# AwesomePeiweiPan/Droid-SLAM_Reserch

Hardware: AMD Instinct MI355X
Metric: BA update iters/sec (2000-edge equivalents; 256 keyframes, 48x64) (higher is better)
Workload: dtype f32; 1 GPU; 256-keyframe / 2000-edge global BA, 48x64, t0=1, lm=1e-5 ep=1e-2 (BASELINE configs[2]); edges_total=2000, solve=fp64 dense Cholesky on device, chol_failed=False

## Files before the change

droid-slam_reserch_amd/csrc/api.hip:

```cpp
#include <hip/hip_runtime.h>
#include <stdarg.h>
#include <stdio.h>

#include <map>
#include <mutex>

#include "../../include/droid_backends_hip.h"
#include "ba_internal.hpp"
#include "graph.hpp"

namespace droid {
int launch_corr_index_forward(const void* volume, const float* coords, void* corr, int B, int H1,
                              int W1, int H2, int W2, int r, int dtype, hipStream_t s);
int launch_corr_pyramid_forward(const void* const* volumes, const float* coords, void* corr, int B, int H1, int W1,
                                int r, int levels, int dtype, hipStream_t s);
int launch_corr_pyramid_forward_slots(const void* const* volumes, const int64_t* slots, long long cap, const float* coords,
                                      void* corr, int B, int H1, int W1, int r, int levels, int dtype, hipStream_t s);
int launch_corr_index_backward(const float* coords, const void* corr_grad, void* volume_grad, int B,
                               int H1, int W1, int H2, int W2, int r, int dtype, hipStream_t s);
int launch_altcorr_pyramid_forward(const void* const* levels_dev, const int64_t* ii, const int64_t* jj,
                                   const float* coords, float* corr, int E, int frames, int H, int W, int C,
                                   int r, int nlevels, int dtype, hipStream_t s);
int launch_altcorr_forward(const void* f1, const void* f2, const float* coords, void* corr, int B,
                           int N, int H1, int W1, int H2, int W2, int C, int r, int dtype,
// ... 483 lines not shown
int droid_ba_status(const void* workspace, void* stream, int* status_out, int* depth_slots_out) {
  if (!workspace) return fail(DROID_E_ARG, "ba_status: null %s", "workspace");
  int hdr[HDR_WORDS];
  hipError_t e = hipMemcpyAsync(hdr, workspace, sizeof(hdr), hipMemcpyDeviceToHost, (hipStream_t)stream);
  if (e == hipSuccess) e = hipStreamSynchronize((hipStream_t)stream);
  if (e != hipSuccess) {
    snprintf(g_err, sizeof(g_err), "ba_status: %s", hipGetErrorString(e));
    return DROID_E_HIP;
  }
  if (status_out) *status_out = hdr[HDR_STATUS];
  if (depth_slots_out) *depth_slots_out = hdr[HDR_M];
  return DROID_OK;
}

int droid_ba_attach_launch_hints(const void* workspace, int* hints) {
  if (!workspace) return fail(DROID_E_ARG, "ba_attach_launch_hints: null %s", "workspace");
  std::lock_guard<std::mutex> lock(g_mirror_mu);
  if (hints) {
    hints[0] = hints[1] = 0;
    g_hint[workspace] = HintState{hints, 0};
  }
  else g_hint.erase(workspace);
  return DROID_OK;
}

int droid_ba_attach_status_mirror(const void* workspace, int* mirror) {
  if (!workspace) return fail(DROID_E_ARG, "ba_attach_status_mirror: null %s", "workspace");
  std::lock_guard<std::mutex> lock(g_mirror_mu);
  if (mirror) g_mirror[workspace] = mirror;
  else g_mirror.erase(workspace);
  return DROID_OK;
}

size_t droid_chol_scratch_doubles(int n) { return CholSystem::scratch_doubles(n); }

int droid_chol_solve(const double* A, const double* b, double* x, int n, double* scratch,
                     int* fail_flag, void* stream) {
  if (n <= 0 || !A || !b || !x || !scratch || !fail_flag) return fail(DROID_E_ARG, "chol_solve: bad %s", "argument");
  hipStream_t s = (hipStream_t)stream;
  const CholSystem c(scratch, n, x, fail_flag);
  launch_chol_pack(A, b, c.S, c.n, c.ld, s);
  launch_chol_solve(c, 0.0, 0.0, s, false);
  return check_hip("chol_solve");
}

int droid_frame_distance(const float* poses, const float* disps, const float* intrinsics,
                         const int64_t* ii, const int64_t* jj, int E, int nbuf, int H, int W,
                         float beta, float* dist, void* stream) {
  if (E < 0 || nbuf <= 0 || H <= 0 || W <= 0) return fail(DROID_E_ARG, "frame_distance: bad %s", "sizes");
  if (E == 0) return DROID_OK;
  if (!poses || !disps || !intrinsics || !ii || !jj || !dist) return fail(DROID_E_ARG, "frame_distance: null %s", "pointer");
  launch_frame_distance(poses, disps, intrinsics, ii, jj, E, nbuf, H, W, beta, dist, (hipStream_t)stream);
  return check_hip("frame_distance");
}

int droid_frame_distance_matrix(const float* poses, const float* disps, const float* intrinsics, int n, int nbuf,
                                int H, int W, float beta, float* dist, void* stream) {
  if (n < 0 || nbuf <= 0 || n > nbuf || H <= 0 || W <= 0) return fail(DROID_E_ARG, "frame_distance_matrix: bad %s", "sizes");
  if (n == 0) return DROID_OK;
  if (!poses || !disps || !intrinsics || !dist) return fail(DROID_E_ARG, "frame_distance_matrix: null %s", "pointer");
  launch_frame_distance_matrix(poses, disps, intrinsics, n, H, W, beta, dist, (hipStream_t)stream);
  return check_hip("frame_distance_matrix");
}

int droid_projmap(const float* poses, const float* disps, const float* intrinsics,
                  const int64_t* ii, const int64_t* jj, int E, int nbuf, int H, int W,
// ... 139 lines not shown
```

droid-slam_reserch_amd/csrc/ba_internal.hpp:

```cpp
#pragma once
#include <hip/hip_runtime.h>
#include <stddef.h>
#include <stdint.h>

namespace droid {

constexpr int LIN_THREADS = 256;
constexpr int LIN_PPT = 2;
constexpr int LIN_CP = LIN_THREADS * LIN_PPT;
constexpr int CHOL_NB = 64;
__host__ __device__ inline int chol_ld(int n) { return (n + 1 + 15) & ~15; }
__host__ __device__ inline size_t chol_flag_words(int n) { return 2 * ((size_t)(n + 1 + CHOL_NB - 1) / CHOL_NB) + 8; }
__host__ __device__ inline int chol_tile_index(int nrb, int bi, int bj) { return bj * nrb - bj * (bj - 1) / 2 + (bi - bj); }
__host__ __device__ inline size_t chol_tiles(int n) {
  const int nb = (n + CHOL_NB - 1) / CHOL_NB, nrb = (n + 1 + CHOL_NB - 1) / CHOL_NB;
  return (size_t)chol_tile_index(nrb, nb, nb);
}
__host__ __device__ inline size_t chol_mbuf_offset(int n) { return ((size_t)(n + CHOL_NB - 1) / CHOL_NB) * CHOL_NB * CHOL_NB; }
__host__ __device__ inline size_t chol_lfin_offset(int n) { return 2 * chol_mbuf_offset(n); }
__host__ __device__ inline size_t chol_ldiag_doubles(int n) { return chol_lfin_offset(n) + chol_tiles(n) * CHOL_NB * CHOL_NB; }

__host__ __device__ inline size_t pk_colbase(int n, int J) {
  return (size_t)CHOL_NB * ((size_t)J * (size_t)(n + 1) - (size_t)CHOL_NB * (size_t)J * (size_t)(J - 1) / 2);
}
__host__ __device__ inline int pk_width(int n, int J) { return (n - CHOL_NB * J) < CHOL_NB ? (n - CHOL_NB * J) : CHOL_NB; }
__host__ __device__ inline size_t pk_total(int n) {
  if (n <= 0) return 0;
  const int nb = (n + CHOL_NB - 1) / CHOL_NB;
  return pk_colbase(n, nb - 1) + (size_t)(n + 1 - CHOL_NB * (nb - 1)) * (size_t)pk_width(n, nb - 1);
}
__host__ __device__ inline size_t pk_index(int n, int gi, int gj) {
  const int J = gj / CHOL_NB;
  return pk_colbase(n, J) + (size_t)(gi - CHOL_NB * J) * (size_t)pk_width(n, J) + (size_t)(gj - CHOL_NB * J);
}
__host__ __device__ inline unsigned pk_index32(int n, int gi, int gj) {
  const int J = gj >> 6, c0 = J << 6;
  const int w = (n - c0) < CHOL_NB ? (n - c0) : CHOL_NB;
  return (unsigned)(CHOL_NB * (J * (n + 1) - (CHOL_NB / 2) * J * (J - 1)) + (gi - c0) * w + (gj - c0));
}

enum { HDR_STATUS = 0, HDR_M = 1, HDR_CHOL_FAIL = 2, HDR_NENT = 3, HDR_NWORK = 4,
       HDR_NC1 = 5, HDR_NC2 = 6,
// ... 55 lines not shown
constexpr int SW_BIG = 512;
constexpr int tri_tiles16(int rows) { return (rows / 16) * (rows / 16 + 1) / 2; }
constexpr int SY_T1 = tri_tiles16(SW_MID), SY_T2 = tri_tiles16(SW_BIG);
constexpr int SY_FOLD_GROUPS = SY_T1 / 4;

inline size_t ba_carve(BaView& v, void* ws, int E, int nbuf, int H, int W, int t0, int t1, int M) {
  v.E = E; v.nbuf = nbuf; v.H = H; v.W = W; v.HW = H * W;
  v.t0 = t0; v.t1 = t1; v.P = t1 - t0; v.M = M;
  v.n = 6 * v.P; v.ld = chol_ld(v.n);
  v.nch = (v.HW + LIN_CP - 1) / LIN_CP;
  v.own0 = 0; v.own1 = nbuf; v.motion_only = 0;
  v.hint = nullptr; v.hint_tag = 0;
  size_t off = 0;
  char* base = static_cast<char*>(ws);
  auto take = [&](size_t bytes) {
    void* p = base ? base + off : nullptr;
    off += (bytes + 255) & ~size_t(255);
    return p;
  };
  v.hdr = static_cast<int*>(take(sizeof(int) * HDR_WORDS));
  v.slot_of = static_cast<int*>(take(sizeof(int) * (nbuf + 1)));
  v.kx = static_cast<int*>(take(sizeof(int) * (nbuf + 1)));
  v.seg_ptr = static_cast<int*>(take(sizeof(int) * (nbuf + 2)));
  v.seg_edge = static_cast<int*>(take(sizeof(int) * (E + 1)));
  v.cursor = static_cast<int*>(take(sizeof(int) * (nbuf + 2)));
  v.ent_ptr = static_cast<int*>(take(sizeof(int) * (nbuf + 2)));
  v.ent_row = static_cast<int*>(take(sizeof(int) * ((size_t)M + E + 1)));
  v.ent_pose = static_cast<int*>(take(sizeof(int) * ((size_t)M + E + 1)));
  v.wk_ptr = static_cast<int*>(take(sizeof(int) * (nbuf + 2)));
  v.order = static_cast<int*>(take(sizeof(int) * (nbuf + 2)));
  v.gt_ptr = static_cast<int*>(take(sizeof(int) * (nbuf + 2)));
  v.cls_list = static_cast<int*>(take(sizeof(int) * 2 * (nbuf + 2)));
  v.xtmp = static_cast<int*>(take(sizeof(int) * 3 * ((size_t)E + 1)));
  v.Hpart = static_cast<float*>(take(sizeof(float) * ((size_t)E * v.nch * 32 + 32)));
  v.Q = static_cast<float*>(take(sizeof(float) * ((size_t)M * v.HW + 4)));
  v.w = static_cast<float*>(take(sizeof(float) * ((size_t)M * v.HW + 4)));
  v.Erows = nullptr;
  v.wide = (M > 0 && (long)E >= 12l * M && (v.HW % 32) == 0) ? 1 : 0;
  v.Ebuf = nullptr;
  if (v.wide) v.Ebuf = static_cast<float*>(take(sizeof(float) * (6 * ((size_t)M + E) * v.HW + 64)));
  v.sy_part[0] = v.sy_part[1] = nullptr;
  v.sy_ns[0] = v.sy_ns[1] = 0;
  if (v.wide) {
    const int stages = v.HW / 32;
    int nsw = (SY_WGS + M - 1) / M, nsb = (256 + 4 * M - 1) / (4 * M);
    nsw = nsw < 2 ? 2 : (nsw > stages ? stages : nsw);
    nsb = nsb < 2 ? 2 : (nsb > stages ? stages : nsb);
    if (nsw > 16) nsw = 16;
    if (nsb > 16) nsb = 16;
    v.sy_ns[0] = nsw; v.sy_ns[1] = nsb;
    v.sy_part[0] = static_cast<float*>(take(sizeof(float) * ((size_t)M * nsw * SY_T1 * 256 + 64)));
    v.sy_part[1] = static_cast<float*>(take(sizeof(float) * ((size_t)M * nsb * SY_T2 * 256 + 64)));
  }
  v.zsplit = 1;
  if (M > 0) {
    const int z = LIN_WGS / (M * v.nch);
    v.zsplit = z < 1 ? 1 : (z > 8 ? 8 : z);
  }
  v.zpart = nullptr;
  if (v.zsplit > 1) v.zpart = static_cast<float*>(take(sizeof(float) * ((size_t)v.zsplit * M * 8 * v.HW + 64)));
  v.s2_split = 1;
  v.Gpart = nullptr;
  if (M > 0) {
    const int ptiles = (v.HW + 63) / 64;
    int ns = S2_WGS / M;
    v.s2_split = ns < 1 ? 1 : (ns > ptiles ? ptiles : ns);
    size_t tiles = (size_t)E * 7 / 4 + (size_t)M + 1;
// ... 15 lines not shown
  return (int)((reinterpret_cast<const char*>(v.bs_flags) - reinterpret_cast<const char*>(v.xsol)) / 4 +
               (long)chol_flag_words(v.n));
}
__host__ __device__ inline int solver_preset_tiles(const BaView& v) { return v.n > 0 ? (int)chol_tiles(v.n) : 0; }

struct BaLaunchPlan {
  int zero_wgs;
  int asm_units;
  dim3 schur2;
  int sf_split;
  dim3 syrk[2], fold;
};
inline BaLaunchPlan ba_launch_plan(const BaView& v) {
  BaLaunchPlan p;
  p.zero_wgs = LIN_ZERO_WGS;
  p.asm_units = v.E > 0 ? v.E + (solver_preset_words(v) + 1023) / 1024 + solver_preset_tiles(v) : 0;
  p.schur2 = dim3(v.M + (p.asm_units + 4 * v.s2_split - 1) / (4 * v.s2_split), v.s2_split);
  const int tiles = (v.HW + SF_TP - 1) / SF_TP, ns = SF_WGS / (v.M > 0 ? v.M : 1);
  p.sf_split = ns < 1 ? 1 : (ns > tiles ? tiles : ns);
  p.syrk[0] = dim3(v.M, v.sy_ns[0], 1);
  p.syrk[1] = dim3(v.M, v.sy_ns[1], 4);
  p.fold = dim3(v.M, SY_FOLD_GROUPS, 2);
  return p;
}

struct CholSystem {
  double* S; int n, ld; double* x; int* flags; double* ldiag; int* fail;
  explicit CholSystem(const BaView& v)
      : S(v.sys), n(v.n), ld(v.ld), x(v.xsol), flags(v.bs_flags), ldiag(v.ldiag), fail(v.hdr + HDR_CHOL_FAIL) {}
  CholSystem(double* scratch, int n, double* x, int* fail);
  static size_t scratch_doubles(int n);
};

void launch_prep(const BaView& v, const int64_t* ii, const int64_t* jj, hipStream_t s);
void launch_unpack_system(const BaView& v, hipStream_t s);
void launch_build_stage(const BaView& v, const BaLaunchPlan& plan, const float* poses, const float* disps,
                        const float* intr, const float* sens, const float* targets, const float* weights,
                        const float* eta, const int64_t* ii, const int64_t* jj, bool motion_only,
                        int stage, hipStream_t s);
void launch_update(const BaView& v, float* poses, float* disps, const float* intr, const float* weights,
                   const int64_t* ii, const int64_t* jj, const double* x, float* dx_out, float* dz_out,
                   bool motion_only, hipStream_t s, int* status_mirror = nullptr);
void launch_chol_preset(const CholSystem& c, hipStream_t s);
bool launch_chol_factor(const CholSystem& c, double lm, double ep, hipStream_t s);
void launch_chol_backsolve(const CholSystem& c, bool factor_single, hipStream_t s);
void launch_chol_solve(const CholSystem& c, double lm, double ep, hipStream_t s, bool preset_done);

void launch_unpack_cols(const BaView& v, int J0, int J1, double lm, double ep, int epoch, hipStream_t s);
bool launch_chol_factor_overlap(const CholSystem& c, const int* ready, int epoch, hipStream_t s);
bool chol_overlap_available(int n);

}
```

droid-slam_reserch_amd/csrc/ba_kernels.hip:

```cpp
#include <hip/hip_runtime.h>
#include <stdint.h>
#include <stdlib.h>

#include "ba_internal.hpp"
#include "se3.hpp"

namespace droid {


__device__ void block_exscan(int* data, int L, int* lds, int* total) {
  const int T = blockDim.x, t = threadIdx.x, lane = t & 63, wave = t >> 6, nw = T >> 6;
  const int per = (L + T - 1) / T;
  const int b = t * per;
  int s = 0;
  for (int k = 0; k < per; k++)
    if (b + k < L) s += data[b + k];
  int incl = s;
#pragma unroll
  for (int off = 1; off < 64; off <<= 1) {
    const int v = __shfl_up(incl, off);
    if (lane >= off) incl += v;
  }
  if (lane == 63) lds[wave] = incl;
  __syncthreads();
  if (wave == 0) {
    int w = (lane < nw) ? lds[lane] : 0;
    int wi = w;
#pragma unroll
    for (int off = 1; off < 64; off <<= 1) {
      const int v = __shfl_up(wi, off);
      if (lane >= off) wi += v;
    }
    if (lane < nw) lds[lane] = wi - w;
    if (lane == nw - 1) *total = wi;
  }
  __syncthreads();
  int run = lds[wave] + incl - s;
  for (int k = 0; k < per; k++)
    if (b + k < L) {
      int v = data[b + k];
      data[b + k] = run;
      run += v;
    }
  __syncthreads();
}

__device__ __forceinline__ float wave_reduce32(float (&v)[32]) {
  const int lane = threadIdx.x & 63;
#pragma unroll
  for (int i = 0; i < 16; i++) {
    const bool hi = lane & 32;
    float keep = hi ? v[2 * i + 1] : v[2 * i];
    float send = hi ? v[2 * i] : v[2 * i + 1];
    v[i] = keep + __shfl_xor(send, 32);
  }
#pragma unroll
  for (int i = 0; i < 8; i++) {
    const bool hi = lane & 16;
    float keep = hi ? v[2 * i + 1] : v[2 * i];
    float send = hi ? v[2 * i] : v[2 * i + 1];
    v[i] = keep + __shfl_xor(send, 16);
  }
#pragma unroll
  for (int i = 0; i < 4; i++) {
    const bool hi = lane & 8;
    float keep = hi ? v[2 * i + 1] : v[2 * i];
    float send = hi ? v[2 * i] : v[2 * i + 1];
    v[i] = keep + __shfl_xor(send, 8);
  }
#pragma unroll
  for (int i = 0; i < 2; i++) {
    const bool hi = lane & 4;
    float keep = hi ? v[2 * i + 1] : v[2 * i];
    float send = hi ? v[2 * i] : v[2 * i + 1];
    v[i] = keep + __shfl_xor(send, 4);
  }
  {
    const bool hi = lane & 2;
    float keep = hi ? v[1] : v[0];
    float send = hi ? v[0] : v[1];
    v[0] = keep + __shfl_xor(send, 2);
  }
  return v[0] + __shfl_xor(v[0], 1);
}

__device__ __forceinline__ int reduce32_index(int lane) {
  return ((lane >> 5) & 1) | (((lane >> 4) & 1) << 1) | (((lane >> 3) & 1) << 2) |
         (((lane >> 2) & 1) << 3) | (((lane >> 1) & 1) << 4);
}

__device__ __forceinline__ double* sys_at(const BaView& v, int gi, int gj) {
  if (v.packed) {
    unsigned idx = pk_index32(v.n, gi, gj);
    asm volatile("" : "+v"(idx));
    return v.psys + idx;
  }
  return v.sys + (size_t)gi * v.ld + gj;
}

constexpr int SLOT_MAXE = 128;
template <typename S>
struct SlotMetaT {
  int e[SLOT_MAXE];
  int pj[SLOT_MAXE];
  int ent[SLOT_MAXE];
  int flag[SLOT_MAXE];
  S T[SLOT_MAXE][12];
};
typedef SlotMetaT<float> SlotMeta;

constexpr int SF_RB = 96;
constexpr int SY_MAXSPLIT = 16;

constexpr int S2_MAXE = 16;
__device__ __forceinline__ int schur_class(int rows, int nedges, int wide) {
  if (nedges <= S2_MAXE) return 0;
  if (!wide || nedges > SLOT_MAXE || rows > SW_BIG) return 3;
  return rows <= SW_MID ? 1 : 2;
}
__device__ __forceinline__ size_t ebuf_index(int e0, int rows, int HW, int row, int k) {
  return (size_t)6 * e0 * HW + ((size_t)(k >> 5) * rows + row) * 32 + (k & 31);
// ... 194 lines not shown
    my3 += (c == 3) ? 1 : 0;
  }
  const int n3 = __syncthreads_count(my3);
  if (t == 0 && vg.hint) {
    __hip_atomic_store(vg.hint + 1, n3, __ATOMIC_RELAXED, __HIP_MEMORY_SCOPE_SYSTEM);
    __hip_atomic_store(vg.hint, vg.hint_tag, __ATOMIC_RELEASE, __HIP_MEMORY_SCOPE_SYSTEM);
  }
  for (int m = t; m < Ms; m += T) {
    const int c = v.wk_ptr[m];
    if (c != 1 && c != 2) continue;
    int pos = 0, after = 0;
    for (int u = 0; u < Ms; u++) {
      const int same = v.wk_ptr[u] == c;
      pos += (same && u < m) ? 1 : 0;
      after += (same && u > m) ? 1 : 0;
    }
    vg.cls_list[(c - 1) * (nbuf + 2) + pos] = m;
    if (after == 0) v.hdr[HDR_NC1 + c - 1] = pos + 1;
  }
  if (INLDS) {
    __syncthreads();
    for (int f = t; f <= nbuf; f += T) {
      vg.slot_of[f] = (f < nbuf) ? v.slot_of[f] : -1;
      vg.kx[f] = v.kx[f];
      vg.seg_ptr[f] = v.seg_ptr[f];
      vg.ent_ptr[f] = v.ent_ptr[f];
      vg.gt_ptr[f] = v.gt_ptr[f];
      vg.order[f] = v.order[f];
    }
    for (int x = t; x < E; x += T) vg.seg_edge[x] = v.seg_edge[x];
  }
}

template <bool DEPTH, bool EROWS, bool ZSPLIT>
__global__ __launch_bounds__(LIN_THREADS, 3) void ba_lin_kernel(
    BaView v, const float* __restrict__ poses, const float* __restrict__ disps,
    const float* __restrict__ intrinsics, const float* __restrict__ disps_sens,
    const float* __restrict__ targets, const float* __restrict__ weights,
    const float* __restrict__ eta, const int64_t* __restrict__ ii, const int64_t* __restrict__ jj, int zero_base) {
  __shared__ float red[2][LIN_THREADS / 64][32];
  __shared__ SlotMetaT<double> sm;
  const int tid = threadIdx.x, lane = tid & 63, wave = tid >> 6;
  const int HW = v.HW, W = v.W;
  const int chunk = blockIdx.y;
  if ((int)blockIdx.x >= zero_base) {
    if (blockIdx.y != 0 || blockIdx.z != 0) return;
    const int nz = (int)gridDim.x - zero_base;
    if (v.packed) {
      double2* p = reinterpret_cast<double2*>(v.psys);
      const size_t n2 = pk_total(v.n) / 2;
      for (size_t c = (size_t)((int)blockIdx.x - zero_base) * LIN_THREADS + tid; c < n2; c += (size_t)nz * LIN_THREADS)
        p[c] = make_double2(0.0, 0.0);
      return;
    }
    for (int row = (int)blockIdx.x - zero_base; row <= v.n; row += nz) {
      double2* p = reinterpret_cast<double2*>(v.sys + (size_t)row * v.ld);
      const int n2 = (row == v.n) ? v.ld / 2 : (row + 2) / 2;
      for (int c = tid; c < n2; c += LIN_THREADS) p[c] = make_double2(0.0, 0.0);
    }
    return;
  }
  int xb, xe, f = -1, m = -1;
  if (DEPTH) {
    if ((int)blockIdx.x >= min(v.hdr[HDR_M], v.M)) return;
    m = v.order[blockIdx.x];
    f = v.kx[m];
    xb = v.seg_ptr[m];
    xe = v.seg_ptr[m + 1];
  } else {
    xb = blockIdx.x;
    xe = xb + 1;
    const int64_t i0 = ii[xb], j0 = jj[xb];
    if (i0 < 0 || i0 >= v.nbuf || j0 < 0 || j0 >= v.nbuf) return;
// ... 1 lines not shown
  const Intr K = {intrinsics[0], intrinsics[1], intrinsics[2], intrinsics[3]};
  int xs = xb, xend = xe;
  if (DEPTH && ZSPLIT) {
    const int per = (xe - xb + (int)gridDim.z - 1) / (int)gridDim.z;
    xs = min(xe, xb + (int)blockIdx.z * per);
    xend = min(xe, xs + per);
  }

  bool emit = false, has_self = false;
  int e0 = 0, erows = 0;
  if (DEPTH && EROWS) {
    e0 = v.ent_ptr[m];
    const int nent = v.ent_ptr[m + 1] - e0;
    erows = 6 * nent;
    const int cls = schur_class(6 * nent + 1, xe - xb, 1);
    emit = (cls == 1 || cls == 2);
    has_self = nent > 0 && (v.ent_row[e0] < v.M);
  }
  float selfacc[LIN_PPT][6];
#pragma unroll
  for (int p = 0; p < LIN_PPT; p++)
#pragma unroll
    for (int n = 0; n < 6; n++) selfacc[p][n] = 0.f;

  int pix[LIN_PPT];
  float disp[LIN_PPT], Cacc[LIN_PPT], wacc[LIN_PPT];
  double X0d[LIN_PPT], X1d[LIN_PPT];
#pragma unroll
  for (int p = 0; p < LIN_PPT; p++) {
    pix[p] = chunk * LIN_CP + p * LIN_THREADS + tid;
    Cacc[p] = 0.f;
    wacc[p] = 0.f;
    disp[p] = 0.f;
    if (DEPTH && pix[p] < HW) disp[p] = disps[(size_t)f * HW + pix[p]];
    const int kk = pix[p] < HW ? pix[p] : 0;
    X0d[p] = ((double)(kk % W) - (double)K.cx) / (double)K.fx;
    X1d[p] = ((double)(kk / W) - (double)K.cy) / (double)K.fy;
  }

  float in_cur[LIN_PPT][4], in_nxt[LIN_PPT][4];
  bool have_next = false;
  auto fetch_edge = [&](int e, float (&dst)[LIN_PPT][4]) {
    const float* tg = targets + (size_t)e * 2 * HW;
    const float* wg = weights + (size_t)e * 2 * HW;
#pragma unroll
    for (int p = 0; p < LIN_PPT; p++) {
      const bool ok = pix[p] < HW;
      const int k = ok ? pix[p] : 0;
      dst[p][0] = ok ? tg[k] : 0.f;
      dst[p][1] = ok ? tg[HW + k] : 0.f;
      dst[p][2] = ok ? wg[k] : 0.f;
      dst[p][3] = ok ? wg[HW + k] : 0.f;
    }
  };
  int buf = 0;
  for (int x = xs; x < xend; x++) {
    if (DEPTH && (x == xs || ((x - xb) % SLOT_MAXE) == 0)) {
      if (x > xs) __syncthreads();
      const int cb = xb + ((x - xb) / SLOT_MAXE) * SLOT_MAXE;
      load_slot_meta(sm, v, poses, jj, f, cb, min(SLOT_MAXE, xe - cb), (EROWS && has_self) ? 1 : 0);
    }
    const int xl = DEPTH ? (x - xb) % SLOT_MAXE : 0;
    const int e = DEPTH ? sm.e[xl] : x;
    const int ix = DEPTH ? f : (int)ii[e];
    double Rt[12];
    bool stereo;
    if (DEPTH) {
#pragma unroll
      for (int n = 0; n < 12; n++) Rt[n] = sm.T[xl][n];
      stereo = sm.flag[xl] != 0;
    } else {
      const int jx = (int)jj[e];
      const RelMat<double> T = rel_pose_mat<double, true>(poses, ix, jx);
#pragma unroll
      for (int n = 0; n < 9; n++) Rt[n] = T.R[n];
#pragma unroll
      for (int n = 0; n < 3; n++) Rt[9 + n] = T.t[n];
      stereo = (ix == jx);
    }
    if (!have_next) fetch_edge(e, in_cur);
    else {
#pragma unroll
      for (int p = 0; p < LIN_PPT; p++)
#pragma unroll
        for (int c = 0; c < 4; c++) in_cur[p][c] = in_nxt[p][c];
    }
    have_next = false;
    if (DEPTH && x + 1 < xend && xl + 1 < SLOT_MAXE) {
      fetch_edge(sm.e[xl + 1], in_nxt);
      have_next = true;
    }
    float acc[32];
#pragma unroll
    for (int k = 0; k < 32; k++) acc[k] = 0.f;
#pragma unroll
    for (int p = 0; p < LIN_PPT; p++) {
      if (pix[p] < HW) {
        const int k = pix[p];
        const float d = DEPTH ? disp[p] : disps[(size_t)ix * HW + k];
        const PixLin L = linearize_pixel_d(K, Rt, Rt + 9, X0d[p], X1d[p], d, in_cur[p][0], in_cur[p][1]);
        float wu = L.valid * (0.001f * in_cur[p][2]);
        float wv = L.valid * (0.001f * in_cur[p][3]);
        if (DEPTH) {
          Cacc[p] += wu * L.Jzu * L.Jzu + wv * L.Jzv * L.Jzv;
          wacc[p] += wu * L.ru * L.Jzu + wv * L.rv * L.Jzv;
        }
        if (stereo) {
          wu = 0.f;
          wv = 0.f;
        }
        int l = 0;
#pragma unroll
        for (int a = 0; a < 6; a++) {
          const float wa_u = wu * L.Ju[a], wa_v = wv * L.Jv[a];
#pragma unroll
          for (int b = 0; b <= a; b++) {
            acc[l] += wa_u * L.Ju[b] + wa_v * L.Jv[b];
            l++;
          }
          acc[21 + a] += wa_u * L.ru + wa_v * L.rv;
        }
        if (DEPTH && EROWS && emit) {
          const float su = wu * L.Jzu, sv = wv * L.Jzv;
          float eij[6];
#pragma unroll
          for (int n = 0; n < 6; n++) eij[n] = su * L.Ju[n] + sv * L.Jv[n];
          const int a = sm.ent[xl];
          if (a >= 0) {
#pragma unroll
            for (int n = 0; n < 6; n++) v.Ebuf[ebuf_index(e0, erows, HW, 6 * a + n, k)] = eij[n];
          }
          if (has_self) {
            float eii[6];
            adjT_mat(Rt, Rt + 9, eij, eii);
#pragma unroll
            for (int n = 0; n < 6; n++) selfacc[p][n] -= eii[n];
          }
        }
      }
    }
    const float tot = wave_reduce32(acc);
    if ((lane & 1) == 0) red[buf][wave][reduce32_index(lane)] = tot;
    __syncthreads();
    if (tid < 32) {
      float s = 0.f;
#pragma unroll
      for (int wv_ = 0; wv_ < LIN_THREADS / 64; wv_++) s += red[buf][wv_][tid];
      v.Hpart[((size_t)e * v.nch + chunk) * 32 + tid] = s;
    }
    buf ^= 1;
  }

  if (DEPTH && ZSPLIT) {
#pragma unroll
    for (int p = 0; p < LIN_PPT; p++) {
      if (pix[p] < HW) {
        float* zp = v.zpart + (((size_t)blockIdx.z * v.M + m) * 8) * HW + pix[p];
        zp[0] = Cacc[p];
        zp[(size_t)HW] = wacc[p];
#pragma unroll
        for (int n = 0; n < 6; n++) zp[(size_t)(2 + n) * HW] = selfacc[p][n];
      }
    }
    return;
  }
  if (DEPTH) {
    const float alpha = 0.05f;
#pragma unroll
    for (int p = 0; p < LIN_PPT; p++) {
      if (pix[p] < HW) {
        const int k = pix[p];
        const size_t o = (size_t)m * HW + k;
        const float sens = disps_sens[(size_t)f * HW + k];
        const float ms = sens > 0.f ? 1.f : 0.f;
        const float C = Cacc[p] + ms * alpha + (1.f - ms) * eta[o];
        const float w = wacc[p] - ms * alpha * (disp[p] - sens);
        v.Q[o] = 1.0f / C;
        v.w[o] = w;
        if (EROWS && emit && has_self) {
#pragma unroll
          for (int n = 0; n < 6; n++) v.Ebuf[ebuf_index(e0, erows, HW, n, k)] = selfacc[p][n];
        }
      }
    }
  }
}

__global__ __launch_bounds__(256) void ba_lin_finish_kernel(BaView v, const float* __restrict__ disps,
                                                            const float* __restrict__ disps_sens,
                                                            const float* __restrict__ eta) {
  if ((int)blockIdx.x >= min(v.hdr[HDR_M], v.M)) return;
  const int m = blockIdx.x, HW = v.HW;
  const int k = blockIdx.y * 256 + threadIdx.x;
  if (k >= HW) return;
  const int f = v.kx[m];
  float s[8] = {0.f, 0.f, 0.f, 0.f, 0.f, 0.f, 0.f, 0.f};
  for (int z = 0; z < v.zsplit; z++) {
    const float* zp = v.zpart + (((size_t)z * v.M + m) * 8) * HW + k;
#pragma unroll
    for (int q = 0; q < 8; q++) s[q] += zp[(size_t)q * HW];
  }
  const float alpha = 0.05f;
  const size_t o = (size_t)m * HW + k;
// ... 9 lines not shown
      for (int n = 0; n < 6; n++) v.Ebuf[ebuf_index(e0, 6 * nent, HW, n, k)] = s[2 + n];
    }
  }
}

struct AssembleScratch {
  double hj[6][6], vj[6], A[6][6], hij[6][6];
};
__device__ __forceinline__ void assemble_unit(const BaView& v, const float* __restrict__ poses, const int64_t* __restrict__ ii,
                                              const int64_t* __restrict__ jj, int e, int t, AssembleScratch& sh) {
  auto& hj = sh.hj; auto& vj = sh.vj; auto& A = sh.A; auto& hij = sh.hij;
  if (e >= v.E) {
    unsigned* w = reinterpret_cast<unsigned*>(v.xsol);
    const int words = solver_preset_words(v);
    const int nw = (words + 1023) / 1024;
    if (e - v.E < nw) {
      for (int i = (e - v.E) * 1024 + t; i < min(words, (e - v.E + 1) * 1024); i += 64) w[i] = 0xFFFFFFFFu;
      if (e == v.E && t == 0) v.hdr[HDR_CHOL_FAIL] = 0;
    } else {
      uint4* q = reinterpret_cast<uint4*>(v.ldiag + chol_lfin_offset(v.n) + (size_t)(e - v.E - nw) * CHOL_NB * CHOL_NB);
      for (int i = t; i < CHOL_NB * CHOL_NB / 2; i += 64) q[i] = make_uint4(0xFFFFFFFFu, 0xFFFFFFFFu, 0xFFFFFFFFu, 0xFFFFFFFFu);
    }
    return;
  }
  const int64_t i64 = ii[e], j64 = jj[e];
  if (i64 < 0 || i64 >= v.nbuf || j64 < 0 || j64 >= v.nbuf) return;
  const int ix = (int)i64, jx = (int)j64;
  if (ix == jx) return;
  const int pi = ix - v.t0, pj = jx - v.t0;
  const bool vi_ok = pi >= 0 && pi < v.P, vj_ok = pj >= 0 && pj < v.P;
  if (!vi_ok && !vj_ok) return;
  if (t < 27) {
    double s = 0.0;
    for (int c = 0; c < v.nch; c++) s += (double)v.Hpart[((size_t)e * v.nch + c) * 32 + t];
    if (t < 21) {
      int a = 0, rem = t;
      while (rem > a) {
        rem -= a + 1;
        a++;
      }
      hj[a][rem] = s;
      hj[rem][a] = s;
    } else {
      vj[t - 21] = s;
    }
  }
  if (t >= 32 && t < 38) {
    const int k = t - 32;
    const RelMat<double> T = rel_pose_mat<double, true>(poses, ix, jx);
    double X[6] = {0.0, 0.0, 0.0, 0.0, 0.0, 0.0}, Y[6];
    X[k] = 1.0;
    adjT_mat(T.R, T.t, X, Y);
    for (int r = 0; r < 6; r++) A[r][k] = Y[r];
  }
  __builtin_amdgcn_wave_barrier();
  asm volatile("s_waitcnt lgkmcnt(0)" ::: "memory");
  const int n = v.n;
  if (t < 36) {
    const int r = t / 6, c = t % 6;
    double s = 0.0;
    for (int k = 0; k < 6; k++) s -= A[r][k] * hj[k][c];
    hij[r][c] = s;
  }
  __builtin_amdgcn_wave_barrier();
  asm volatile("s_waitcnt lgkmcnt(0)" ::: "memory");
  if (t < 36) {
    const int r = t / 6, c = t % 6;
// ... 1087 lines not shown
  }
}
__global__ void ba_set_ready_kernel(int* __restrict__ ready, int b0, int b1, int epoch) {
  const int b = b0 + (int)threadIdx.x;
  if (b < b1) __hip_atomic_store(ready + b, epoch, __ATOMIC_RELEASE, __HIP_MEMORY_SCOPE_AGENT);
}

void launch_unpack_system(const BaView& v, hipStream_t s) {
  if (v.n <= 0) return;
  const int nb = (v.n + CHOL_NB - 1) / CHOL_NB;
  hipLaunchKernelGGL(ba_unpack_kernel<false>, dim3(min((v.n + 8) / 8, 64), nb), dim3(256), 0, s, v, 0, 0.0, 0.0);
}

void launch_unpack_cols(const BaView& v, int J0, int J1, double lm, double ep, int epoch, hipStream_t s) {
  if (J1 <= J0) return;
  hipLaunchKernelGGL(ba_unpack_kernel<true>, dim3(min((v.n + 8 - CHOL_NB * J0) / 8, 64), J1 - J0), dim3(256), 0, s, v, J0, lm, ep);
  hipLaunchKernelGGL(ba_set_ready_kernel, dim3(1), dim3(64), 0, s, v.ov_ready, J0, J1, epoch);
}

void launch_prep(const BaView& v, const int64_t* ii, const int64_t* jj, hipStream_t s) {
  const size_t lds_bytes = sizeof(int) * prep_lds_ints(v.nbuf, v.E);
  static bool attr_set = false;
  if (lds_bytes <= 150 * 1024) {
    if (!attr_set) {
      (void)hipFuncSetAttribute((const void*)ba_prep_kernel<true>, hipFuncAttributeMaxDynamicSharedMemorySize, 150 * 1024);
      attr_set = true;
    }
    hipLaunchKernelGGL(ba_prep_kernel<true>, dim3(1), dim3(1024), lds_bytes, s, v, ii, jj);
  } else {
    hipLaunchKernelGGL(ba_prep_kernel<false>, dim3(1), dim3(1024), 0, s, v, ii, jj);
  }
}

void launch_build_stage(const BaView& v, const BaLaunchPlan& plan, const float* poses, const float* disps,
                        const float* intr, const float* sens, const float* targets, const float* weights,
                        const float* eta, const int64_t* ii, const int64_t* jj, bool motion_only,
                        int stage, hipStream_t s) {
  const bool depth = !motion_only && v.M > 0;
  switch (stage) {
    case 0:
      if (depth) {
        const dim3 g(v.M + plan.zero_wgs, v.nch, v.zsplit), b(LIN_THREADS);
        const auto lin = v.wide ? (v.zsplit > 1 ? ba_lin_kernel<true, true, true> : ba_lin_kernel<true, true, false>)
                                : (v.zsplit > 1 ? ba_lin_kernel<true, false, true> : ba_lin_kernel<true, false, false>);
        hipLaunchKernelGGL(lin, g, b, 0, s, v, poses, disps, intr, sens, targets, weights, eta, ii, jj, v.M);
        if (v.zsplit > 1)
          hipLaunchKernelGGL(ba_lin_finish_kernel, dim3(v.M, (v.HW + 255) / 256), dim3(256), 0, s, v, disps, sens, eta);
      } else if (v.E > 0) {
        hipLaunchKernelGGL((ba_lin_kernel<false, false, false>), dim3(v.E + plan.zero_wgs, v.nch), dim3(LIN_THREADS), 0, s, v, poses,
                           disps, intr, sens, targets, weights, eta, ii, jj, v.E);
      } else {
        if (v.packed) (void)hipMemsetAsync(v.psys, 0, sizeof(double) * pk_total(v.n), s);
        else (void)hipMemsetAsync(v.sys, 0, sizeof(double) * (size_t)(v.n + 1) * v.ld, s);
      }
      break;
    case 1:
      if (v.E > 0 && !depth)
        hipLaunchKernelGGL(ba_assemble_kernel, dim3(plan.asm_units), dim3(64), 0, s, v, poses, ii, jj);
      break;
    case 2:
      if (depth) {
        const int wide = v.wide;
        hipLaunchKernelGGL(ba_schur2_kernel, plan.schur2, dim3(256), 0, s, v, poses, disps, intr, weights, ii, jj,
                           wide, plan.asm_units);
        hipLaunchKernelGGL(ba_schur_fold_kernel, dim3(v.M), dim3(1024), 0, s, v, poses, jj, v.s2_split);
        bool none3 = false;
        if (v.hint) {
          const int tag = __atomic_load_n(v.hint, __ATOMIC_ACQUIRE);
          none3 = tag == v.hint_tag && __atomic_load_n(v.hint + 1, __ATOMIC_RELAXED) == 0;
        }
        if (!none3)
          hipLaunchKernelGGL(ba_schur_fused_kernel, dim3(v.M, plan.sf_split), dim3(256), 0, s, v, poses, disps,
                             intr, weights, ii, jj, wide);
        if (wide) {
          hipLaunchKernelGGL((ba_syrk3_kernel<SW_MID, 12, 1, 1, true, true>), plan.syrk[0], dim3(768), 0, s, v);
          hipLaunchKernelGGL((ba_syrk3_kernel<SW_BIG, 8, 2, 4, false, false>), plan.syrk[1], dim3(512), 0, s, v);
          hipLaunchKernelGGL(ba_syrk_fold_kernel, plan.fold, dim3(256), 0, s, v, v.M * v.sy_ns[0], v.M * v.sy_ns[1]);
        }
      }
      break;
  }
}
// ... 12 lines not shown
```

droid-slam_reserch_amd/droid_backends/_lib.py:

```python
from __future__ import annotations

import ctypes
import os

_HERE = os.path.dirname(os.path.abspath(__file__))
LIB_PATH = os.environ.get("DROID_HIP_LIB") or os.path.join(_HERE, "libdroid_backends_hip.so")

SYMBOLS = [
    "droid_abi_version", "droid_last_error",
    "droid_corr_index_forward", "droid_corr_index_backward", "droid_corr_pyramid_forward",
    "droid_corr_volume_pyramid", "droid_corr_pyramid_forward_slots", "droid_corr_volume_pyramid_slots",
    "droid_altcorr_forward", "droid_altcorr_backward", "droid_altcorr_pyramid_forward",
    "droid_altcorr_pyramid_forward_f16",
    "droid_ba_workspace_bytes", "droid_ba", "droid_ba_prepare", "droid_ba_build", "droid_ba_build_packed",
    "droid_ba_packed_system", "droid_ba_unpack_system",
    "droid_ba_overlap_available", "droid_ba_overlap_plan", "droid_ba_unpack_chunk", "droid_ba_solve_update_overlap",
    "droid_ba_solve_update", "droid_ba_profile_iteration", "droid_ba_system", "droid_ba_status",
    "droid_ba_attach_status_mirror", "droid_ba_attach_launch_hints", "droid_chol_solve", "droid_chol_scratch_doubles", "droid_reproject_motion",
    "droid_frame_distance", "droid_frame_distance_matrix", "droid_projmap", "droid_iproj", "droid_depth_filter",
    "droid_proximity_workspace_bytes", "droid_proximity_edges",
    "droid_cvx_upsample",
    "droid_graph_mean_workspace_bytes", "droid_graph_mean",
]

DROID_F16, DROID_F32, DROID_F64 = 0, 1, 2

_lib = None


class DroidBackendError(RuntimeError):
    pass


def load() -> ctypes.CDLL:
    global _lib
    if _lib is not None:
        return _lib
    if not os.path.exists(LIB_PATH):
        raise DroidBackendError(
            f"{LIB_PATH} is missing: build the HIP extension first "
            "(python -c 'import __graft_entry__ as g; g.build()' or droid-slam_reserch_amd/csrc/build.sh). "
            "There is no CPU fallback.")
    lib = ctypes.CDLL(LIB_PATH)
    for s in SYMBOLS:
        if not hasattr(lib, s):
            raise DroidBackendError(f"{LIB_PATH} does not export {s}")
    c_int, c_float, vp, sz = ctypes.c_int, ctypes.c_float, ctypes.c_void_p, ctypes.c_size_t
    lib.droid_abi_version.restype = c_int
    lib.droid_last_error.restype = ctypes.c_char_p
    lib.droid_corr_index_forward.argtypes = [vp, vp, vp] + [c_int] * 7 + [vp]
    lib.droid_corr_index_backward.argtypes = [vp, vp, vp] + [c_int] * 7 + [vp]
    lib.droid_corr_pyramid_forward.argtypes = [ctypes.POINTER(vp), vp, vp] + [c_int] * 6 + [vp]
    lib.droid_corr_volume_pyramid.argtypes = ([vp, vp, vp, ctypes.POINTER(vp)] + [c_int] * 7
                                              + [ctypes.c_int64, ctypes.c_int64, c_int, vp])
    lib.droid_corr_pyramid_forward_slots.argtypes = ([ctypes.POINTER(vp), vp, vp, vp, c_int, ctypes.c_int64]
# ... 11 lines not shown
    lib.droid_ba_build.argtypes = [vp] * 9 + [c_int] * 8 + [vp, sz, vp]
    lib.droid_ba_build_packed.argtypes = [vp] * 9 + [c_int] * 8 + [vp, sz, vp]
    lib.droid_ba_packed_system.argtypes = [vp] + [c_int] * 7 + [ctypes.POINTER(sz)]
    lib.droid_ba_packed_system.restype = vp
    lib.droid_ba_unpack_system.argtypes = [c_int] * 8 + [vp, sz, vp]
    lib.droid_ba_solve_update.argtypes = [vp] * 6 + [c_int] * 7 + [c_float, c_float, c_int, vp, vp, vp, sz, vp]
    lib.droid_ba_overlap_available.argtypes = [c_int, c_int]
    lib.droid_ba_overlap_plan.argtypes = [c_int, c_int, c_int, ctypes.POINTER(c_int), ctypes.POINTER(sz)]
    lib.droid_ba_unpack_chunk.argtypes = [c_int] * 9 + [c_float, c_float, c_int, vp, sz, vp]
    lib.droid_ba_solve_update_overlap.argtypes = [vp] * 6 + [c_int] * 9 + [vp, vp, vp, sz, vp]
    lib.droid_ba_profile_iteration.argtypes = [vp] * 9 + [c_int] * 7 + [c_float, c_float, c_int, vp, sz, vp, vp]
    lib.droid_ba_system.argtypes = [vp] + [c_int] * 7 + [ctypes.POINTER(sz)]
    lib.droid_ba_system.restype = vp
    lib.droid_ba_status.argtypes = [vp, vp, ctypes.POINTER(c_int), ctypes.POINTER(c_int)]
    lib.droid_ba_attach_status_mirror.argtypes = [vp, vp]
    lib.droid_ba_attach_launch_hints.argtypes = [vp, vp]
    lib.droid_chol_solve.argtypes = [vp, vp, vp, c_int, vp, vp, vp]
    lib.droid_reproject_motion.argtypes = [vp, vp, vp, c_int, vp, vp, vp, c_int, c_int, c_int, c_int, vp, vp, vp, vp]
    lib.droid_chol_scratch_doubles.argtypes = [c_int]
    lib.droid_chol_scratch_doubles.restype = ctypes.c_size_t
    lib.droid_frame_distance.argtypes = [vp] * 5 + [c_int] * 4 + [c_float, vp, vp]
    lib.droid_frame_distance_matrix.argtypes = [vp] * 3 + [c_int] * 4 + [c_float, vp, vp]
    lib.droid_projmap.argtypes = [vp] * 5 + [c_int] * 4 + [vp, vp, vp]
    lib.droid_iproj.argtypes = [vp] * 3 + [c_int] * 3 + [vp, vp]
    lib.droid_depth_filter.argtypes = [vp] * 5 + [c_int] * 4 + [vp, vp]
    lib.droid_proximity_workspace_bytes.argtypes = [c_int] * 5
    lib.droid_proximity_workspace_bytes.restype = sz
    lib.droid_proximity_edges.argtypes = ([vp] + [c_int] * 7 + [c_float, c_int, c_int, vp, vp, c_int, vp, vp, c_int,
                                                                vp, c_int, vp, vp, sz, vp])
    lib.droid_cvx_upsample.argtypes = [vp] * 4 + [c_int] * 6 + [vp]
    lib.droid_graph_mean_workspace_bytes.argtypes = [c_int, c_int]
    lib.droid_graph_mean_workspace_bytes.restype = sz
    lib.droid_graph_mean.argtypes = [vp, vp, vp, c_int, ctypes.c_int64] + [c_int] * 4 + [vp, vp, sz, vp]
    for s in SYMBOLS[2:]:
        if s not in ("droid_ba_workspace_bytes", "droid_ba_system", "droid_ba_packed_system", "droid_chol_scratch_doubles",
                     "droid_proximity_workspace_bytes", "droid_graph_mean_workspace_bytes"):
            getattr(lib, s).restype = c_int
    if lib.droid_abi_version() != 1:
        raise DroidBackendError("ABI version mismatch")
    _lib = lib
    return lib


def check(rc: int, what: str):
    if rc != 0:
        msg = load().droid_last_error().decode("utf-8", "replace")
        raise RuntimeError(f"droid_backends.{what} failed (rc={rc}): {msg}")
```

include/droid_backends_hip.h:

```cpp
#ifndef DROID_BACKENDS_HIP_H
#define DROID_BACKENDS_HIP_H

#include <stddef.h>
#include <stdint.h>

#ifdef __cplusplus
extern "C" {
#endif

#define DROID_ABI_VERSION 1

#define DROID_OK 0
#define DROID_E_ARG (-1)
#define DROID_E_WORKSPACE (-2)
#define DROID_E_HIP (-3)

#define DROID_F16 0
#define DROID_F32 1
#define DROID_F64 2

int droid_abi_version(void);
const char *droid_last_error(void);


// ... 62 lines not shown
int droid_ba_unpack_system(int E, int nbuf, int H, int W, int M, int t0, int t1, int motion_only,
                           void *workspace, size_t workspace_bytes, void *stream);

int droid_ba_overlap_available(int t0, int t1);
int droid_ba_overlap_plan(int t0, int t1, int max_chunks, int *nchunks_out, size_t *packed_offsets);
int droid_ba_unpack_chunk(int E, int nbuf, int H, int W, int M, int t0, int t1, int chunk, int max_chunks, float lm,
                          float ep, int epoch, void *workspace, size_t workspace_bytes, void *stream);
int droid_ba_solve_update_overlap(float *poses, float *disps, const float *intrinsics, const float *weights,
                                  const int64_t *ii, const int64_t *jj, int E, int nbuf, int H, int W, int M,
                                  int t0, int t1, int epoch, int motion_only, float *dx_out, float *dz_out,
                                  void *workspace, size_t workspace_bytes, void *stream);

int droid_ba_solve_update(float *poses, float *disps, const float *intrinsics, const float *weights,
                          const int64_t *ii, const int64_t *jj, int E, int nbuf, int H, int W, int M,
                          int t0, int t1, float lm, float ep, int motion_only, float *dx_out,
                          float *dz_out, void *workspace, size_t workspace_bytes, void *stream);

int droid_ba_profile_iteration(float *poses, float *disps, const float *intrinsics,
                               const float *disps_sens, const float *targets, const float *weights,
                               const float *eta, const int64_t *ii, const int64_t *jj, int E,
                               int nbuf, int H, int W, int M, int t0, int t1, float lm, float ep,
                               int motion_only, void *workspace, size_t workspace_bytes,
                               void *stream, float *stage_ms);

double *droid_ba_system(void *workspace, int E, int nbuf, int H, int W, int t0, int t1, int M,
                        size_t *n_elements);

int droid_ba_status(const void *workspace, void *stream, int *status_out, int *depth_slots_out);

int droid_ba_attach_status_mirror(const void *workspace, int *mirror);

int droid_ba_attach_launch_hints(const void *workspace, int *hints);

size_t droid_chol_scratch_doubles(int n);
int droid_chol_solve(const double *A, const double *b, double *x, int n, double *scratch,
                     int *fail_flag, void *stream);


int droid_frame_distance(const float *poses, const float *disps, const float *intrinsics,
                         const int64_t *ii, const int64_t *jj, int E, int nbuf, int H, int W,
                         float beta, float *dist, void *stream);

int droid_frame_distance_matrix(const float *poses, const float *disps, const float *intrinsics, int n,
                                int nbuf, int H, int W, float beta, float *dist, void *stream);

int droid_projmap(const float *poses, const float *disps, const float *intrinsics,
                  const int64_t *ii, const int64_t *jj, int E, int nbuf, int H, int W,
                  float *coords, float *valid, void *stream);

int droid_reproject_motion(const float *poses, const float *disps, const float *intrinsics, int intr_stride,
                           const int64_t *ii, const int64_t *jj, const float *target, int E, int nbuf, int H,
                           int W, float *coords, float *valid, float *motn, void *stream);

int droid_iproj(const float *poses, const float *disps, const float *intrinsics, int nm, int H,
                int W, float *points, void *stream);

int droid_depth_filter(const float *poses, const float *disps, const float *intrinsics,
                       const int64_t *ix, const float *thresh, int num, int nbuf, int H, int W,
                       float *counter, void *stream);


int droid_cvx_upsample(const float *data, const int64_t *ix, const void *mask, float *out, int n, int nbuf_in,
                       int nbuf_out, int H, int W, int mask_dtype, void *stream);


#define DROID_GRAPH_MEAN_MAX_RANGE 16384
// ... 17 lines not shown
```

Before: 1966 iters/s.

## Use permlane/DPP wave reduction, drop block sync in BA linearization

Rewrites the 32-value wave reduction to use permlane32/16 swaps and DPP row moves instead of shuffle-xor, which removes LDS round trips. Each wave now writes its own partial Hessian slice to global memory, so the per-chunk shared-memory reduction and __syncthreads are gone. The downstream assembly kernel sums the per-wave partials instead. A FULL template variant drops the per-pixel bounds checks when HW is a multiple of the chunk size. The trade-off is a larger Hpart buffer with more global writes and reads, plus a test entry point for checking the reduction.

```diff
diff --git a/droid-slam_reserch_amd/csrc/api.hip b/droid-slam_reserch_amd/csrc/api.hip
--- a/droid-slam_reserch_amd/csrc/api.hip
+++ b/droid-slam_reserch_amd/csrc/api.hip
@@ -539,6 +539,12 @@
   return DROID_OK;
 }
 
+int droid_test_wave_reduce32(const float* in, float* out, void* stream) {
+  if (!in || !out) return fail(DROID_E_ARG, "test_wave_reduce32: null %s", "pointer");
+  launch_wave_reduce32_test(in, out, (hipStream_t)stream);
+  return check_hip("test_wave_reduce32");
+}
+
 size_t droid_chol_scratch_doubles(int n) { return CholSystem::scratch_doubles(n); }
 
 int droid_chol_solve(const double* A, const double* b, double* x, int n, double* scratch,
diff --git a/droid-slam_reserch_amd/csrc/ba_internal.hpp b/droid-slam_reserch_amd/csrc/ba_internal.hpp
--- a/droid-slam_reserch_amd/csrc/ba_internal.hpp
+++ b/droid-slam_reserch_amd/csrc/ba_internal.hpp
@@ -8,6 +8,7 @@
 constexpr int LIN_THREADS = 256;
 constexpr int LIN_PPT = 2;
 constexpr int LIN_CP = LIN_THREADS * LIN_PPT;
+constexpr int LIN_WAVES = LIN_THREADS / 64;
 constexpr int CHOL_NB = 64;
 __host__ __device__ inline int chol_ld(int n) { return (n + 1 + 15) & ~15; }
 __host__ __device__ inline size_t chol_flag_words(int n) { return 2 * ((size_t)(n + 1 + CHOL_NB - 1) / CHOL_NB) + 8; }
@@ -129,7 +130,7 @@
   v.gt_ptr = static_cast<int*>(take(sizeof(int) * (nbuf + 2)));
   v.cls_list = static_cast<int*>(take(sizeof(int) * 2 * (nbuf + 2)));
   v.xtmp = static_cast<int*>(take(sizeof(int) * 3 * ((size_t)E + 1)));
-  v.Hpart = static_cast<float*>(take(sizeof(float) * ((size_t)E * v.nch * 32 + 32)));
+  v.Hpart = static_cast<float*>(take(sizeof(float) * ((size_t)E * v.nch * LIN_WAVES * 32 + 32)));
   v.Q = static_cast<float*>(take(sizeof(float) * ((size_t)M * v.HW + 4)));
   v.w = static_cast<float*>(take(sizeof(float) * ((size_t)M * v.HW + 4)));
   v.Erows = nullptr;
@@ -211,6 +212,7 @@
   static size_t scratch_doubles(int n);
 };
 
+void launch_wave_reduce32_test(const float* in, float* out, hipStream_t s);
 void launch_prep(const BaView& v, const int64_t* ii, const int64_t* jj, hipStream_t s);
 void launch_unpack_system(const BaView& v, hipStream_t s);
 void launch_build_stage(const BaView& v, const BaLaunchPlan& plan, const float* poses, const float* disps,
diff --git a/droid-slam_reserch_amd/csrc/ba_kernels.hip b/droid-slam_reserch_amd/csrc/ba_kernels.hip
--- a/droid-slam_reserch_amd/csrc/ba_kernels.hip
+++ b/droid-slam_reserch_amd/csrc/ba_kernels.hip
@@ -45,48 +45,57 @@
   __syncthreads();
 }
 
+template <int CTRL, int BANKS>
+__device__ __forceinline__ float dpp_move(float old, float src) {
+  return __int_as_float(__builtin_amdgcn_update_dpp(__float_as_int(old), __float_as_int(src), CTRL, 0xf, BANKS, false));
+}
 __device__ __forceinline__ float wave_reduce32(float (&v)[32]) {
+  constexpr int ROW_SHL4 = 0x104, ROW_SHR4 = 0x114, ROW_ROR8 = 0x128, QUAD_XOR2 = 0x4E, QUAD_XOR1 = 0xB1;
   const int lane = threadIdx.x & 63;
 #pragma unroll
   for (int i = 0; i < 16; i++) {
-    const bool hi = lane & 32;
-    float keep = hi ? v[2 * i + 1] : v[2 * i];
-    float send = hi ? v[2 * i] : v[2 * i + 1];
-    v[i] = keep + __shfl_xor(send, 32);
+    const auto r = __builtin_amdgcn_permlane32_swap(__float_as_uint(v[2 * i]), __float_as_uint(v[2 * i + 1]), false, false);
+    v[i] = __uint_as_float(r[0]) + __uint_as_float(r[1]);
   }
 #pragma unroll
   for (int i = 0; i < 8; i++) {
-    const bool hi = lane & 16;
-    float keep = hi ? v[2 * i + 1] : v[2 * i];
-    float send = hi ? v[2 * i] : v[2 * i + 1];
-    v[i] = keep + __shfl_xor(send, 16);
+    const auto r = __builtin_amdgcn_permlane16_swap(__float_as_uint(v[2 * i]), __float_as_uint(v[2 * i + 1]), false, false);
+    v[i] = __uint_as_float(r[0]) + __uint_as_float(r[1]);
   }
 #pragma unroll
   for (int i = 0; i < 4; i++) {
-    const bool hi = lane & 8;
-    float keep = hi ? v[2 * i + 1] : v[2 * i];
-    float send = hi ? v[2 * i] : v[2 * i + 1];
-    v[i] = keep + __shfl_xor(send, 8);
+    const float a = dpp_move<ROW_ROR8, 0x3>(v[2 * i + 1], v[2 * i]);
+    const float b = dpp_move<ROW_ROR8, 0xC>(v[2 * i], v[2 * i + 1]);
+    v[i] = a + b;
   }
 #pragma unroll
   for (int i = 0; i < 2; i++) {
-    const bool hi = lane & 4;
-    float keep = hi ? v[2 * i + 1] : v[2 * i];
-    float send = hi ? v[2 * i] : v[2 * i + 1];
-    v[i] = keep + __shfl_xor(send, 4);
+    const float a = dpp_move<ROW_SHL4, 0x5>(v[2 * i + 1], v[2 * i]);
+    const float b = dpp_move<ROW_SHR4, 0xA>(v[2 * i], v[2 * i + 1]);
+    v[i] = a + b;
   }
   {
     const bool hi = lane & 2;
     float keep = hi ? v[1] : v[0];
     float send = hi ? v[0] : v[1];
-    v[0] = keep + __shfl_xor(send, 2);
-  }
-  return v[0] + __shfl_xor(v[0], 1);
+    v[0] = keep + dpp_move<QUAD_XOR2, 0xF>(send, send);
+  }
+  return v[0] + dpp_move<QUAD_XOR1, 0xF>(v[0], v[0]);
 }
 
 __device__ __forceinline__ int reduce32_index(int lane) {
   return ((lane >> 5) & 1) | (((lane >> 4) & 1) << 1) | (((lane >> 3) & 1) << 2) |
          (((lane >> 2) & 1) << 3) | (((lane >> 1) & 1) << 4);
+}
+
+__global__ __launch_bounds__(64) void wave_reduce32_test_kernel(const float* __restrict__ in, float* __restrict__ out) {
+  float v[32];
+#pragma unroll
+  for (int k = 0; k < 32; k++) v[k] = in[threadIdx.x * 32 + k];
+  out[threadIdx.x] = wave_reduce32(v);
+}
+void launch_wave_reduce32_test(const float* in, float* out, hipStream_t s) {
+  hipLaunchKernelGGL(wave_reduce32_test_kernel, dim3(1), dim3(64), 0, s, in, out);
 }
 
 __device__ __forceinline__ double* sys_at(const BaView& v, int gi, int gj) {
@@ -347,13 +356,12 @@
   }
 }
 
-template <bool DEPTH, bool EROWS, bool ZSPLIT>
+template <bool DEPTH, bool EROWS, bool ZSPLIT, bool FULL>
 __global__ __launch_bounds__(LIN_THREADS, 3) void ba_lin_kernel(
     BaView v, const float* __restrict__ poses, const float* __restrict__ disps,
     const float* __restrict__ intrinsics, const float* __restrict__ disps_sens,
     const float* __restrict__ targets, const float* __restrict__ weights,
     const float* __restrict__ eta, const int64_t* __restrict__ ii, const int64_t* __restrict__ jj, int zero_base) {
-  __shared__ float red[2][LIN_THREADS / 64][32];
   __shared__ SlotMetaT<double> sm;
   const int tid = threadIdx.x, lane = tid & 63, wave = tid >> 6;
   const int HW = v.HW, W = v.W;
@@ -421,8 +429,8 @@
     Cacc[p] = 0.f;
     wacc[p] = 0.f;
     disp[p] = 0.f;
-    if (DEPTH && pix[p] < HW) disp[p] = disps[(size_t)f * HW + pix[p]];
-    const int kk = pix[p] < HW ? pix[p] : 0;
+    if (DEPTH && (FULL || pix[p] < HW)) disp[p] = disps[(size_t)f * HW + pix[p]];
+    const int kk = (FULL || pix[p] < HW) ? pix[p] : 0;
     X0d[p] = ((double)(kk % W) - (double)K.cx) / (double)K.fx;
     X1d[p] = ((double)(kk / W) - (double)K.cy) / (double)K.fy;
   }
@@ -434,7 +442,7 @@
     const float* wg = weights + (size_t)e * 2 * HW;
 #pragma unroll
     for (int p = 0; p < LIN_PPT; p++) {
-      const bool ok = pix[p] < HW;
+      const bool ok = FULL || pix[p] < HW;
       const int k = ok ? pix[p] : 0;
       dst[p][0] = ok ? tg[k] : 0.f;
       dst[p][1] = ok ? tg[HW + k] : 0.f;
@@ -442,7 +450,6 @@
       dst[p][3] = ok ? wg[HW + k] : 0.f;
     }
   };
-  int buf = 0;
   for (int x = xs; x < xend; x++) {
     if (DEPTH && (x == xs || ((x - xb) % SLOT_MAXE) == 0)) {
       if (x > xs) __syncthreads();
@@ -484,7 +491,7 @@
     for (int k = 0; k < 32; k++) acc[k] = 0.f;
 #pragma unroll
     for (int p = 0; p < LIN_PPT; p++) {
-      if (pix[p] < HW) {
+      if (FULL ? (chunk * LIN_CP + p * LIN_THREADS < HW) : (pix[p] < HW)) {
         const int k = pix[p];
         const float d = DEPTH ? disp[p] : disps[(size_t)ix * HW + k];
         const PixLin L = linearize_pixel_d(K, Rt, Rt + 9, X0d[p], X1d[p], d, in_cur[p][0], in_cur[p][1]);
@@ -529,21 +536,13 @@
       }
     }
     const float tot = wave_reduce32(acc);
-    if ((lane & 1) == 0) red[buf][wave][reduce32_index(lane)] = tot;
-    __syncthreads();
-    if (tid < 32) {
-      float s = 0.f;
-#pragma unroll
-      for (int wv_ = 0; wv_ < LIN_THREADS / 64; wv_++) s += red[buf][wv_][tid];
-      v.Hpart[((size_t)e * v.nch + chunk) * 32 + tid] = s;
-    }
-    buf ^= 1;
+    if ((lane & 1) == 0) v.Hpart[(((size_t)e * v.nch + chunk) * LIN_WAVES + wave) * 32 + reduce32_index(lane)] = tot;
   }
 
   if (DEPTH && ZSPLIT) {
 #pragma unroll
     for (int p = 0; p < LIN_PPT; p++) {
-      if (pix[p] < HW) {
+      if (FULL || pix[p] < HW) {
         float* zp = v.zpart + (((size_t)blockIdx.z * v.M + m) * 8) * HW + pix[p];
         zp[0] = Cacc[p];
         zp[(size_t)HW] = wacc[p];
@@ -557,7 +556,7 @@
     const float alpha = 0.05f;
 #pragma unroll
     for (int p = 0; p < LIN_PPT; p++) {
-      if (pix[p] < HW) {
+      if (FULL || pix[p] < HW) {
         const int k = pix[p];
         const size_t o = (size_t)m * HW + k;
         const float sens = disps_sens[(size_t)f * HW + k];
@@ -633,7 +632,13 @@
   if (!vi_ok && !vj_ok) return;
   if (t < 27) {
     double s = 0.0;
-    for (int c = 0; c < v.nch; c++) s += (double)v.Hpart[((size_t)e * v.nch + c) * 32 + t];
+    for (int c = 0; c < v.nch; c++) {
+      const float* hp = v.Hpart + ((size_t)e * v.nch + c) * LIN_WAVES * 32 + t;
+      float s32 = 0.f;
+#pragma unroll
+      for (int wv_ = 0; wv_ < LIN_WAVES; wv_++) s32 += hp[wv_ * 32];
+      s += (double)s32;
+    }
     if (t < 21) {
       int a = 0, rem = t;
       while (rem > a) {
@@ -1787,22 +1792,32 @@
   }
 }
 
+template <bool FULL>
+static auto lin_kernel_of(bool wide, bool zsplit) {
+  return wide ? (zsplit ? ba_lin_kernel<true, true, true, FULL> : ba_lin_kernel<true, true, false, FULL>)
+              : (zsplit ? ba_lin_kernel<true, false, true, FULL> : ba_lin_kernel<true, false, false, FULL>);
+}
+static auto lin_kernel_of(bool wide, bool zsplit, bool full) {
+  return full ? lin_kernel_of<true>(wide, zsplit) : lin_kernel_of<false>(wide, zsplit);
+}
+
 void launch_build_stage(const BaView& v, const BaLaunchPlan& plan, const float* poses, const float* disps,
                         const float* intr, const float* sens, const float* targets, const float* weights,
                         const float* eta, const int64_t* ii, const int64_t* jj, bool motion_only,
                         int stage, hipStream_t s) {
   const bool depth = !motion_only && v.M > 0;
+  const bool full = v.HW % LIN_CP == 0;
   switch (stage) {
     case 0:
       if (depth) {
         const dim3 g(v.M + plan.zero_wgs, v.nch, v.zsplit), b(LIN_THREADS);
-        const auto lin = v.wide ? (v.zsplit > 1 ? ba_lin_kernel<true, true, true> : ba_lin_kernel<true, true, false>)
-                                : (v.zsplit > 1 ? ba_lin_kernel<true, false, true> : ba_lin_kernel<true, false, false>);
+        const auto lin = lin_kernel_of(v.wide != 0, v.zsplit > 1, full);
         hipLaunchKernelGGL(lin, g, b, 0, s, v, poses, disps, intr, sens, targets, weights, eta, ii, jj, v.M);
         if (v.zsplit > 1)
           hipLaunchKernelGGL(ba_lin_finish_kernel, dim3(v.M, (v.HW + 255) / 256), dim3(256), 0, s, v, disps, sens, eta);
       } else if (v.E > 0) {
-        hipLaunchKernelGGL((ba_lin_kernel<false, false, false>), dim3(v.E + plan.zero_wgs, v.nch), dim3(LIN_THREADS), 0, s, v, poses,
+        const auto lin = full ? ba_lin_kernel<false, false, false, true> : ba_lin_kernel<false, false, false, false>;
+        hipLaunchKernelGGL(lin, dim3(v.E + plan.zero_wgs, v.nch), dim3(LIN_THREADS), 0, s, v, poses,
                            disps, intr, sens, targets, weights, eta, ii, jj, v.E);
       } else {
         if (v.packed) (void)hipMemsetAsync(v.psys, 0, sizeof(double) * pk_total(v.n), s);
diff --git a/droid-slam_reserch_amd/droid_backends/_lib.py b/droid-slam_reserch_amd/droid_backends/_lib.py
--- a/droid-slam_reserch_amd/droid_backends/_lib.py
+++ b/droid-slam_reserch_amd/droid_backends/_lib.py
@@ -21,6 +21,7 @@
     "droid_proximity_workspace_bytes", "droid_proximity_edges",
     "droid_cvx_upsample",
     "droid_graph_mean_workspace_bytes", "droid_graph_mean",
+    "droid_test_wave_reduce32",
 ]
 
 DROID_F16, DROID_F32, DROID_F64 = 0, 1, 2
@@ -98,6 +99,7 @@
     lib.droid_graph_mean_workspace_bytes.argtypes = [c_int, c_int]
     lib.droid_graph_mean_workspace_bytes.restype = sz
     lib.droid_graph_mean.argtypes = [vp, vp, vp, c_int, ctypes.c_int64] + [c_int] * 4 + [vp, vp, sz, vp]
+    lib.droid_test_wave_reduce32.argtypes = [vp, vp, vp]
     for s in SYMBOLS[2:]:
         if s not in ("droid_ba_workspace_bytes", "droid_ba_system", "droid_ba_packed_system", "droid_chol_scratch_doubles",
                      "droid_proximity_workspace_bytes", "droid_graph_mean_workspace_bytes"):
diff --git a/include/droid_backends_hip.h b/include/droid_backends_hip.h
--- a/include/droid_backends_hip.h
+++ b/include/droid_backends_hip.h
@@ -118,6 +118,8 @@
 
 int droid_ba_attach_launch_hints(const void *workspace, int *hints);
 
+int droid_test_wave_reduce32(const float *in, float *out, void *stream);
+
 size_t droid_chol_scratch_doubles(int n);
 int droid_chol_solve(const double *A, const double *b, double *x, int n, double *scratch,
                      int *fail_flag, void *stream);
```

New measurement: 1997 iters/s (median of 6 runs). 1.02x the previous value.
